# atomicarchitects/equiformer

Hardware: NVIDIA H100
Metric: edges/sec fwd+bwd, QM9 Lmax=2 batch (higher is better)
Workload: dtype f32

## Files before the change

equiformer_b200/csrc/eqf_fused.cu:

```cuda
#include <cuda.h>
#include <cuda_runtime.h>

#include <cstdint>
#include <mutex>
#include <string>
#include <vector>

#include "eqf_common.cuh"
#include "eqf_tc.cuh"

namespace eqf {
namespace fused {

using namespace tc;

constexpr int BM = 128;
constexpr int BKT = kKTile;
constexpr int kRowBytes = BKT * 4;
constexpr int kProducerWarp = 4;
constexpr int kHelperWarp0 = 6, kHelperWarps = 2, kHelperThreads = kHelperWarps * 32;
constexpr int kConsumerWarps = 8;
constexpr int kDtpWarp0 = 12, kDtpWarps = 16, kDtpSets = 2, kDtpSetWarps = kDtpWarps / kDtpSets;
constexpr int kDtpSetThreads = kDtpSetWarps * 32;
constexpr int kThreads = (kDtpWarp0 + kDtpWarps) * 32;
constexpr int kMaxBN = 64;
constexpr int kMaxPaths = 16;
constexpr int kMaxTileEdges = 136;
constexpr int kMetaInts = 2 * kMaxTileEdges;
constexpr int kMaxStages = 8;
constexpr int kMaxKTiles = 32;

struct FPath {
  int d1, d2;
  int xb, mul;
  int y_off, w_off;
  int cg_off;
  int koff;
  int m_off;
  unsigned long long nz;
};

struct FArgs {
  const float* x[EQF_MAX_BLOCKS];
  const float* x2[EQF_MAX_BLOCKS];
  const long long* src;
  const long long* dst;
  const float* y;
  const float* w;
  const float* w_offset;
  const float* cg;
  float* C;
  long long ldc;
  long long E, M;
  int d_y, W, w_shared, d3, n_paths, m_row, K, N;
  int n_tile, n_blocks;
  long long m_blocks;
  long long* dbg;
  int n_op, n_raw, op_bytes, w_tile_off, w_box_rows, tab_bytes, m_buf_floats, y_buf_floats, cg_floats;
  unsigned char kt_path[kMaxKTiles];
  FPath paths[kMaxPaths];
};

__device__ __forceinline__ void stamp(const FArgs& a, int role, int& n) {
  if (a.dbg != nullptr && blockIdx.x == 0 && n < 2048) a.dbg[role * 2048 + n] = clock64();
  ++n;
}


template <int BN>
struct FSmem {
  static constexpr int kABytes = BM * kRowBytes;
  static constexpr int kBBytes = BN * kRowBytes;
  static constexpr int kBarBytes = 1024;
  static constexpr int kBudget = 227 * 1024 - 1024;
};

__device__ __forceinline__ float4 ld4(const float* p) { return __ldg(reinterpret_cast<const float4*>(p)); }
__device__ __forceinline__ void addv(float4& a, const float4& b) { a.x += b.x; a.y += b.y; a.z += b.z; a.w += b.w; }
__device__ __forceinline__ void mulv(float4& a, const float4& b) { a.x *= b.x; a.y *= b.y; a.z *= b.z; a.w *= b.w; }
__device__ __forceinline__ void fs(float4& a, const float4& x, float m) {
  a.x = fmaf(x.x, m, a.x); a.y = fmaf(x.y, m, a.y); a.z = fmaf(x.z, m, a.z); a.w = fmaf(x.w, m, a.w);
}

struct Ring {
  int n, idx;
  uint32_t ph;
  __device__ __forceinline__ Ring(int n_) : n(n_), idx(0), ph(0) {}
  __device__ __forceinline__ void next() { if (++idx == n) { idx = 0; ph ^= 1u; } }
};

struct KtWaits { uint64_t* raw_free; uint32_t raw_ph; uint64_t* op_full; uint32_t op_ph; };

template <int D1, int D3, bool DIAG>
__device__ __forceinline__ void dtp_ktile(const FArgs& a, const FPath& p, int ch0, int t, long long e0, int n_e, long long row0,
                                          const int* __restrict__ src_s, const int* __restrict__ dst_s, uint32_t m_addr,
                                          uint32_t raw_addr, uint32_t w_tile, const KtWaits& wt) {
  constexpr int NM = (D1 * D3 + 3) / 4;
  const int c8 = t & 7;
  const int ch = ch0 + c8 * 4;
  const bool gather = a.src != nullptr;
  const float* xa = a.x[p.xb];
  const float* xb = a.x2[p.xb];
  const long long row_floats = (long long)D1 * p.mul;
  float4 woff = make_float4(0.f, 0.f, 0.f, 0.f);
  if (a.w_offset != nullptr) woff = ld4(a.w_offset + p.w_off + ch);
  bool waited = false;
  int el = t >> 3;
#pragma unroll 1
  do {
    const bool active = el < n_e;
    const int els = active ? el : 0;
    const long long e = e0 + els;
    const long long rs = gather ? (long long)src_s[els] : e;
    const float* xp = xa + rs * row_floats + ch;
    float4 x[D1];
#pragma unroll
    for (int i = 0; i < D1; ++i) x[i] = ld4(xp + i * p.mul);
    if (xb != nullptr) {
      const float* xq = xb + (long long)dst_s[els] * row_floats + ch;
      float4 x2[D1];
#pragma unroll
      for (int i = 0; i < D1; ++i) x2[i] = ld4(xq + i * p.mul);
#pragma unroll
      for (int i = 0; i < D1; ++i) addv(x[i], x2[i]);
    }
    if (!waited) {
      waited = true;
      mbar_wait_hint(wt.raw_free, wt.raw_ph);
      if (wt.op_full) mbar_wait_hint(wt.op_full, wt.op_ph);
    }
    if (!active) break;
    float4 wv = w_tile != 0 ? lds128(w_tile + (uint32_t)el * 128u + (uint32_t)c8 * 16u) : ld4(a.w + p.w_off + ch);
    addv(wv, woff);
    float m[NM * 4];
    const uint32_t ma = m_addr + (uint32_t)(el * a.m_row + p.m_off) * 4u;
#pragma unroll
    for (int q = 0; q < NM; ++q) {
      const float4 v = lds128(ma + (uint32_t)q * 16u);
      m[4 * q] = v.x; m[4 * q + 1] = v.y; m[4 * q + 2] = v.z; m[4 * q + 3] = v.w;
    }
    float4 f[D3];
    if constexpr (DIAG) {
#pragma unroll
      for (int k = 0; k < D3; ++k) {
        f[k] = x[k];
        mulv(f[k], wv);
        f[k].x *= m[k * D3 + k]; f[k].y *= m[k * D3 + k]; f[k].z *= m[k * D3 + k]; f[k].w *= m[k * D3 + k];
      }
    } else {
#pragma unroll
      for (int k = 0; k < D3; ++k) f[k] = make_float4(0.f, 0.f, 0.f, 0.f);
#pragma unroll
      for (int i = 0; i < D1; ++i) {
#pragma unroll
        for (int k = 0; k < D3; ++k) fs(f[k], x[i], m[i * D3 + k]);
      }
#pragma unroll
      for (int k = 0; k < D3; ++k) mulv(f[k], wv);
    }
    const int rbase = (int)(e * D3 - row0);
#pragma unroll
    for (int k = 0; k < D3; ++k) {
      const int row = rbase + k;
      if ((unsigned)row < (unsigned)BM) sts128(raw_addr + (uint32_t)row * 128u + (uint32_t)((c8 ^ (row & 7)) << 4), f[k]);
    }
    el += kDtpSetThreads / 8;
  } while (el < n_e);
}

template <int D3>
__device__ __forceinline__ void dtp_ktile_d1(const FArgs& a, const FPath& p, int ch0, int t, long long e0, int n_e, long long row0,
                                             const int* src_s, const int* dst_s, uint32_t m_addr, uint32_t raw_addr,
                                             uint32_t w_tile, const KtWaits& wt) {
  if (p.d2 == 1 && p.d1 == D3) {
    dtp_ktile<D3, D3, true>(a, p, ch0, t, e0, n_e, row0, src_s, dst_s, m_addr, raw_addr, w_tile, wt);
    return;
  }
  switch (p.d1) {
    case 1: dtp_ktile<1, D3, false>(a, p, ch0, t, e0, n_e, row0, src_s, dst_s, m_addr, raw_addr, w_tile, wt); break;
    case 3: dtp_ktile<3, D3, false>(a, p, ch0, t, e0, n_e, row0, src_s, dst_s, m_addr, raw_addr, w_tile, wt); break;
    case 5: dtp_ktile<5, D3, false>(a, p, ch0, t, e0, n_e, row0, src_s, dst_s, m_addr, raw_addr, w_tile, wt); break;
    default: dtp_ktile<7, D3, false>(a, p, ch0, t, e0, n_e, row0, src_s, dst_s, m_addr, raw_addr, w_tile, wt); break;
  }
}


template <int BN, int D3>
__global__ void __launch_bounds__(kThreads, 1)
dtp_gemm_fwd_kernel(const __grid_constant__ CUtensorMap map_bhi, const __grid_constant__ CUtensorMap map_blo,
                    const __grid_constant__ CUtensorMap map_w, const __grid_constant__ FArgs a) {
  using S = FSmem<BN>;
  const int n_op = a.n_op, n_raw = a.n_raw;
  extern __shared__ uint8_t smem_raw[];
  uint8_t* smem = reinterpret_cast<uint8_t*>((reinterpret_cast<uintptr_t>(smem_raw) + 1023) & ~uintptr_t(1023));
  uint8_t* op_base = smem;
  uint8_t* raw_base = smem + (size_t)n_op * a.op_bytes;
  uint8_t* tab_base = raw_base + (size_t)n_raw * S::kABytes;
  int4* mdesc = reinterpret_cast<int4*>(tab_base + 2 * a.tab_bytes);
  float* cg_s = reinterpret_cast<float*>(reinterpret_cast<uint8_t*>(mdesc) + ((a.m_row * 16 + 127) & ~127));
  uint64_t* bars = reinterpret_cast<uint64_t*>(reinterpret_cast<uint8_t*>(cg_s) + ((a.cg_floats * 4 + 127) & ~127));
  uint64_t* op_full = bars;
  uint64_t* op_empty = bars + kMaxStages;
  uint64_t* raw_ready = bars + 2 * kMaxStages;
  uint64_t* raw_free = bars + 3 * kMaxStages;
  uint64_t* tab_ready = bars + 4 * kMaxStages;
  uint64_t* tab_free = tab_ready + 2;

  const int warp = threadIdx.x >> 5, lane = threadIdx.x & 31;
  const int k_tiles = a.K / BKT;
  constexpr int d3 = D3;
  const long long n_tiles_total = a.m_blocks * a.n_blocks;
  const bool w_tma = !a.w_shared;

  if (threadIdx.x == kProducerWarp * 32) {
    prefetch_map(&map_bhi); prefetch_map(&map_blo);
    if (w_tma) prefetch_map(&map_w);
    for (int s = 0; s < kMaxStages; ++s) {
      mbar_init(&op_full[s], 1);
      mbar_init(&op_empty[s], kConsumerWarps);
      mbar_init(&raw_ready[s], kDtpSetWarps);
      mbar_init(&raw_free[s], kConsumerWarps);
    }
    for (int b = 0; b < 2; ++b) {
      mbar_init(&tab_ready[b], kHelperWarps);
      mbar_init(&tab_free[b], kDtpWarps);
    }
    asm volatile("fence.mbarrier_init.release.cluster;" ::: "memory");
  }
  __syncthreads();

  if (warp < 4 || (warp >= 8 && warp < kDtpWarp0)) {
    reg_alloc<80>();
    const int row_wg = (warp < 4 ? 0 : 64) + (warp & 3) * 16;
    const bool stamper = threadIdx.x == 0;
    Ring op(n_op), raw(n_raw);
    int n_stamp = 0;
    for (long long tile = blockIdx.x; tile < n_tiles_total; tile += gridDim.x) {
      const long long mb = tile / a.n_blocks;
      const int nb = (int)(tile % a.n_blocks);
      float acc[BN / 2];
#pragma unroll
      for (int i = 0; i < BN / 2; ++i) acc[i] = 0.f;
      for (int kt = 0; kt < k_tiles; ++kt, op.next(), raw.next()) {
        mbar_wait_hint(&op_full[op.idx], op.ph);
        mbar_wait_hint(&raw_ready[raw.idx], raw.ph);
        if (stamper) stamp(a, 1, n_stamp);
        const uint32_t raw_tile = smem_u32(raw_base + (size_t)raw.idx * S::kABytes);
        const uint32_t st = smem_u32(op_base + (size_t)op.idx * a.op_bytes);
#pragma unroll
        for (int half = 0; half < 2; ++half) {
          uint32_t hi[8], lo[8];
          load_a_split(raw_tile, row_wg, lane, hi, lo, 2 * half);
          if (half == 1) {
            __syncwarp();
            if (lane == 0) mbar_arrive(&raw_free[raw.idx]);
          }
          mma_ktile_3xtf32<BN>(acc, hi, lo, st, st + S::kBBytes, 2 * half);
          wgmma_wait<0>();
        }
        __syncwarp();
        if (lane == 0) mbar_arrive(&op_empty[op.idx]);
        if (stamper) stamp(a, 1, n_stamp);
      }
      store_acc<BN>(acc, a.C, a.ldc, mb * BM + row_wg, a.M, nb * BN, a.N, lane, false);
      if (stamper) stamp(a, 3, n_stamp);
    }
  } else if (warp < 8) {
    reg_dealloc<56>();
    if (warp == kProducerWarp) {
      if (lane == 0) {
        Ring op(n_op);
        int n_stamp = 0;
        const uint32_t tx = (uint32_t)(2 * S::kBBytes) + (w_tma ? (uint32_t)(a.w_box_rows * kRowBytes) : 0u);
        for (long long tile = blockIdx.x; tile < n_tiles_total; tile += gridDim.x) {
          const long long mb = tile / a.n_blocks;
          const int nb = (int)(tile % a.n_blocks);
          const int e0 = (int)((mb * BM) / d3);
          for (int kt = 0; kt < k_tiles; ++kt, op.next()) {
            mbar_wait_hint(&op_empty[op.idx], op.ph ^ 1);
            stamp(a, 0, n_stamp);
            uint8_t* st = op_base + (size_t)op.idx * a.op_bytes;
            mbar_expect_tx(&op_full[op.idx], tx);
            tma_load_2d(st, &map_bhi, kt * BKT, nb * BN, &op_full[op.idx]);
            tma_load_2d(st + S::kBBytes, &map_blo, kt * BKT, nb * BN, &op_full[op.idx]);
            if (w_tma) {
              const FPath& p = a.paths[a.kt_path[kt]];
              tma_load_2d(st + a.w_tile_off, &map_w, p.w_off + (kt * BKT - p.koff), e0, &op_full[op.idx]);
            }
          }
        }
      }
    } else if (warp >= kHelperWarp0) {
      const int ht = threadIdx.x - kHelperWarp0 * 32;
      const int m_row = a.m_row, d_y = a.d_y;
      {
        int off = 0;
        for (int pi = 0; pi < a.n_paths; ++pi) {
          const FPath& p = a.paths[pi];
          const int n = p.d1 * p.d2 * d3;
          for (int i = ht; i < n; i += kHelperThreads) cg_s[off + i] = __ldg(a.cg + p.cg_off + i);
          off += n;
        }
        for (int q = ht; q < m_row; q += kHelperThreads) {
          int pi = 0, cg0 = 0;
          for (int j = 1; j < a.n_paths; ++j) if (q >= a.paths[j].m_off) pi = j;
          for (int j = 0; j < pi; ++j) cg0 += a.paths[j].d1 * a.paths[j].d2 * d3;
          const FPath& p = a.paths[pi];
          const int r = q - p.m_off;
          const int i = r / d3, k = r - i * d3;
          if (i < p.d1) mdesc[q] = make_int4(cg0 + i * p.d2 * d3 + k, p.y_off, p.d2, 0);
          else mdesc[q] = make_int4(0, 0, 0, 0);
        }
        named_barrier(2, kHelperThreads);
      }
      const uint32_t cg_addr = smem_u32(cg_s);
      uint32_t tile_it = 0;
      int n_stamp = 0;
      for (long long tile = blockIdx.x; tile < n_tiles_total; tile += gridDim.x, ++tile_it) {
        const long long mb = tile / a.n_blocks;
        const long long row0 = mb * BM;
        const long long e0 = row0 / d3;
        long long e1 = (row0 + BM - 1) / d3 + 1;
        if (e1 > a.E) e1 = a.E;
        const int n_e = (int)(e1 - e0);
        const int b = tile_it & 1;
        mbar_wait_hint(&tab_free[b], ((tile_it >> 1) & 1) ^ 1);
        if (ht == 0) stamp(a, 5, n_stamp);
        float* mw = reinterpret_cast<float*>(tab_base + b * a.tab_bytes);
        float* ybuf = mw + a.m_buf_floats;
        int* ss = reinterpret_cast<int*>(ybuf + a.y_buf_floats);
        int* ds = ss + kMaxTileEdges;
        if (a.src != nullptr) {
          for (int i = ht; i < n_e; i += kHelperThreads) {
            ss[i] = (int)a.src[e0 + i];
            ds[i] = a.dst != nullptr ? (int)a.dst[e0 + i] : 0;
          }
        }
        for (int i = ht; i < n_e * d_y; i += kHelperThreads) ybuf[i] = __ldg(a.y + e0 * d_y + i);
        named_barrier(2, kHelperThreads);
        const uint32_t y_addr = smem_u32(ybuf);
        for (int q = ht; q < m_row; q += kHelperThreads) {
          const int4 dsc = mdesc[q];
          float cgr[kMaxD];
#pragma unroll
          for (int j = 0; j < kMaxD; ++j) cgr[j] = j < dsc.z ? lds32(cg_addr + (uint32_t)(dsc.x + j * d3) * 4u) : 0.f;
#pragma unroll 4
          for (int el = 0; el < n_e; ++el) {
            const uint32_t ya = y_addr + (uint32_t)(el * d_y + dsc.y) * 4u;
            float m = 0.f;
#pragma unroll
            for (int j = 0; j < kMaxD; ++j)
              if (j < dsc.z) m = fmaf(cgr[j], lds32(ya + (uint32_t)j * 4u), m);
            mw[el * m_row + q] = m;
          }
        }
        __syncwarp();
        if (lane == 0) mbar_arrive(&tab_ready[b]);
        if (ht == 0) stamp(a, 5, n_stamp);
      }
    }
  } else {
    const int dt = threadIdx.x - kDtpWarp0 * 32;
    const int set = (warp - kDtpWarp0) / kDtpSetWarps;
    const int t = dt - set * kDtpSetThreads;
    Ring op(n_op), raw(n_raw);
    uint32_t it = 0, tile_it = 0;
    int n_stamp = 0;
    const bool stamper = (t == 0 && set == 0);
    for (long long tile = blockIdx.x; tile < n_tiles_total; tile += gridDim.x, ++tile_it) {
      const long long mb = tile / a.n_blocks;
      const long long row0 = mb * BM;
      const long long e0 = row0 / d3;
      long long e1 = (row0 + BM - 1) / d3 + 1;
      if (e1 > a.E) e1 = a.E;
      const int n_e = (int)(e1 - e0);
      const int b = tile_it & 1;
      mbar_wait_hint(&tab_ready[b], (tile_it >> 1) & 1);
      if (stamper) stamp(a, 4, n_stamp);
      const float* mw = reinterpret_cast<const float*>(tab_base + b * a.tab_bytes);
      const float* ybuf = mw + a.m_buf_floats;
      const int* src_s = reinterpret_cast<const int*>(ybuf + a.y_buf_floats);
      const int* dst_s = src_s + kMaxTileEdges;
      const uint32_t m_addr = smem_u32(mw);
      for (int kt = 0; kt < k_tiles; ++kt, ++it, op.next(), raw.next()) {
        if ((int)(it & 1) != set) continue;
        const FPath& p = a.paths[a.kt_path[kt]];
        const int ch0 = kt * BKT - p.koff;
        const uint32_t raw_addr = smem_u32(raw_base + (size_t)raw.idx * S::kABytes);
        const uint32_t w_tile = w_tma ? smem_u32(op_base + (size_t)op.idx * a.op_bytes) + (uint32_t)a.w_tile_off : 0u;
        KtWaits wt;
        wt.raw_free = &raw_free[raw.idx]; wt.raw_ph = raw.ph ^ 1;
        wt.op_full = w_tma ? &op_full[op.idx] : nullptr; wt.op_ph = op.ph;
        if (stamper) stamp(a, 4, n_stamp);
        dtp_ktile_d1<D3>(a, p, ch0, t, e0, n_e, row0, src_s, dst_s, m_addr, raw_addr, w_tile, wt);
        __syncwarp();
        if (lane == 0) mbar_arrive(&raw_ready[raw.idx]);
        if (stamper) stamp(a, 4, n_stamp);
      }
      __syncwarp();
      if (lane == 0) mbar_arrive(&tab_free[b]);
    }
  }
}

template <int D1, int D3>
__device__ __forceinline__ void group_ktile(const FArgs& a, const FPath& p, int ch0, int el, int c8, long long e,
                                            const float* __restrict__ me, float* __restrict__ out) {
  const int ch = ch0 + c8 * 4;
  float4 wv = ld4(a.w + (a.w_shared ? 0 : e * a.W) + p.w_off + ch);
  if (a.w_offset != nullptr) addv(wv, ld4(a.w_offset + p.w_off + ch));
  const long long row_floats = (long long)D1 * p.mul;
  const long long rs = a.src != nullptr ? a.src[e] : e;
  const float* xp = a.x[p.xb] + rs * row_floats + ch;
  float4 x[D1];
#pragma unroll
  for (int i = 0; i < D1; ++i) x[i] = ld4(xp + i * p.mul);
  if (a.x2[p.xb] != nullptr) {
    const float* xq = a.x2[p.xb] + a.dst[e] * row_floats + ch;
#pragma unroll
    for (int i = 0; i < D1; ++i) addv(x[i], ld4(xq + i * p.mul));
  }
#pragma unroll
  for (int i = 0; i < D1; ++i) mulv(x[i], wv);
#pragma unroll
  for (int k = 0; k < D3; ++k) {
    float4 f = make_float4(0.f, 0.f, 0.f, 0.f);
#pragma unroll
    for (int i = 0; i < D1; ++i)
      if ((p.nz >> (i * D3 + k)) & 1ull) fs(f, x[i], me[i * D3 + k]);
    *reinterpret_cast<float4*>(out + (e * D3 + k) * a.K + p.koff + ch) = f;
  }
}

template <int D3>
__global__ void __launch_bounds__(256) dtp_group_forward_kernel(const __grid_constant__ FArgs a, float* __restrict__ out) {
  extern __shared__ float msm[];
  const int t = threadIdx.x, el = t >> 3, c8 = t & 7;
  const int m_row = a.m_row;
  for (long long eb = (long long)blockIdx.x * 32; eb < a.E; eb += (long long)gridDim.x * 32) {
    const int n_e = (int)((a.E - eb) < 32 ? (a.E - eb) : 32);
    __syncthreads();
    for (int idx = t; idx < n_e * m_row; idx += 256) {
      const int ee = idx / m_row, q = idx - ee * m_row;
      int pi = 0;
      for (int j = 1; j < a.n_paths; ++j) if (q >= a.paths[j].m_off) pi = j;
      const FPath& p = a.paths[pi];
      const int r = q - p.m_off;
      const int i = r / D3, k = r - i * D3;
      const float* cg = a.cg + p.cg_off + i * p.d2 * D3 + k;
      const float* yv = a.y + (eb + ee) * a.d_y + p.y_off;
      float m = 0.f;
      for (int j = 0; j < (i < p.d1 ? p.d2 : 0); ++j) m = fmaf(__ldg(cg + j * D3), __ldg(yv + j), m);
      msm[idx] = m;
    }
    __syncthreads();
    if (el < n_e) {
      const long long e = eb + el;
      for (int pi = 0; pi < a.n_paths; ++pi) {
        const FPath& p = a.paths[pi];
        const float* me = msm + el * m_row + p.m_off;
        for (int ch0 = 0; ch0 < p.mul; ch0 += BKT) {
          switch (p.d1) {
            case 1: group_ktile<1, D3>(a, p, ch0, el, c8, e, me, out); break;
            case 3: group_ktile<3, D3>(a, p, ch0, el, c8, e, me, out); break;
            case 5: group_ktile<5, D3>(a, p, ch0, el, c8, e, me, out); break;
            default: group_ktile<7, D3>(a, p, ch0, el, c8, e, me, out); break;
          }
        }
      }
    }
  }
}

__global__ void split_transpose_kernel(const float* __restrict__ w, long long ldw, float* __restrict__ hi,
                                       float* __restrict__ lo, long long N, long long K) {
  const long long n_el = N * K;
  for (long long i = (long long)blockIdx.x * blockDim.x + threadIdx.x; i < n_el; i += (long long)gridDim.x * blockDim.x) {
    const long long n = i / K, k = i - n * K;
    const float v = w[k * ldw + n];
    const float h = tf32_rn(v);
    hi[i] = h;
    lo[i] = tf32_rn(v - h);
  }
}

template <int BN, int D3>
static int launch_fwd_d3(const CUtensorMap& mh, const CUtensorMap& ml, const CUtensorMap& mw, FArgs& a, cudaStream_t s) {
  using S = FSmem<BN>;
  const int n_e_max = BM / a.d3 + 2;
  a.w_box_rows = a.w_shared ? 0 : n_e_max;
  a.w_tile_off = 2 * S::kBBytes;
  a.op_bytes = (a.w_tile_off + a.w_box_rows * kRowBytes + 1023) & ~1023;
  a.m_buf_floats = (n_e_max * a.m_row + 31) & ~31;
  a.y_buf_floats = (n_e_max * a.d_y + 31) & ~31;
  a.cg_floats = 0;
  for (int i = 0; i < a.n_paths; ++i) a.cg_floats += a.paths[i].d1 * a.paths[i].d2 * a.d3;
  a.tab_bytes = ((a.m_buf_floats + a.y_buf_floats) * 4 + kMetaInts * 4 + 127) & ~127;
  const int fixed = 2 * a.tab_bytes + ((a.m_row * 16 + 127) & ~127) + ((a.cg_floats * 4 + 127) & ~127) + S::kBarBytes;
  int n_raw = 0, n_op = 0;
  for (int r = 4; r >= 2 && n_raw == 0; --r) {
    const int o = (S::kBudget - fixed - r * S::kABytes) / a.op_bytes;
    if (o >= r || (r == 2 && o >= 2)) { n_raw = r; n_op = o; }
  }
  if (n_raw == 0) { set_error("fused DTP: the tile does not fit shared memory"); return EQF_ERR_UNSUPPORTED; }
  if (n_op > kMaxStages) n_op = kMaxStages;
  a.n_raw = n_raw; a.n_op = n_op;
  const int total = n_op * a.op_bytes + n_raw * S::kABytes + fixed + 1024;
  static std::mutex mtx;
  static int attr_bytes = 0;
  {
    std::lock_guard<std::mutex> lock(mtx);
    if (total > attr_bytes) {
      cudaError_t e = cudaFuncSetAttribute(dtp_gemm_fwd_kernel<BN, D3>, cudaFuncAttributeMaxDynamicSharedMemorySize, total);
      if (e != cudaSuccess) return check_cuda(e, "dtp_gemm_fwd smem attribute");
      attr_bytes = total;
    }
  }
  const int sms = device_sms();
  const long long tiles = a.m_blocks * a.n_blocks;
  const int grid = (int)(tiles < sms ? tiles : sms);
  dtp_gemm_fwd_kernel<BN, D3><<<grid, kThreads, total, s>>>(mh, ml, mw, a);
  return check_cuda(cudaGetLastError(), "dtp_gemm_fwd_kernel launch");
}

template <int BN>
static int launch_fwd(const CUtensorMap& mh, const CUtensorMap& ml, const CUtensorMap& mw, FArgs& a, cudaStream_t s) {
  switch (a.d3) {
    case 1: return launch_fwd_d3<BN, 1>(mh, ml, mw, a, s);
    case 3: return launch_fwd_d3<BN, 3>(mh, ml, mw, a, s);
    case 5: return launch_fwd_d3<BN, 5>(mh, ml, mw, a, s);
    default: return launch_fwd_d3<BN, 7>(mh, ml, mw, a, s);
  }
}

static int collect_paths(const EqfPlan* plan, int group, FArgs& a) {
  const PlanHdr& h = plan->hdr;
  if (group < 0 || group >= h.n_out) { set_error("fused DTP: output group out of range"); return EQF_ERR_INVALID; }
  const PathDev* pd = reinterpret_cast<const PathDev*>(plan->blob.data() + h.off_paths);
  std::vector<const PathDev*> ps;
  for (int p = 0; p < h.n_paths; ++p) if (pd[p].og == group) ps.push_back(&pd[p]);
  for (size_t i = 0; i < ps.size(); ++i)
    for (size_t j = i; j > 0 && ps[j]->koff < ps[j - 1]->koff; --j) std::swap(ps[j], ps[j - 1]);
  if (ps.empty() || (int)ps.size() > kMaxPaths) { set_error("fused DTP: unsupported number of paths in the group"); return EQF_ERR_UNSUPPORTED; }
  int koff = 0, m_off = 0;
  for (size_t i = 0; i < ps.size(); ++i) {
    const PathDev& s = *ps[i];
    if (s.d1 > kMaxD || s.d2 > kMaxD || s.d3 > kMaxD) {
      set_error("fused DTP: degree-4 paths are not supported (2l+1 <= 7)");
      return EQF_ERR_UNSUPPORTED;
    }
    if (s.koff != koff || s.mul % BKT != 0) {
      set_error("fused DTP: group channels must be covered by paths of multiplicity % 32 == 0");
      return EQF_ERR_UNSUPPORTED;
    }
    FPath& f = a.paths[i];
    f.d1 = s.d1; f.d2 = s.d2; f.xb = s.xb; f.mul = s.mul; f.y_off = s.y_off; f.w_off = s.w_off; f.cg_off = s.cg_off;
    f.koff = s.koff; f.m_off = m_off;
    f.nz = 0;
    const float* cgp = reinterpret_cast<const float*>(plan->blob.data() + h.off_cg) + s.cg_off;
    for (int ii = 0; ii < s.d1; ++ii)
      for (int kk = 0; kk < s.d3; ++kk) {
        bool any = false;
        for (int jj = 0; jj < s.d2; ++jj) any = any || cgp[(ii * s.d2 + jj) * s.d3 + kk] != 0.0f;
        if (any) f.nz |= 1ull << (ii * s.d3 + kk);
      }
    for (int c = 0; c < s.mul / BKT; ++c) {
      if (koff / BKT + c >= kMaxKTiles) { set_error("fused DTP: output group wider than 1024 channels"); return EQF_ERR_UNSUPPORTED; }
      a.kt_path[koff / BKT + c] = (unsigned char)i;
    }
    koff += s.mul;
    m_off += (s.d1 * s.d3 + 3) & ~3;
  }
  a.n_paths = (int)ps.size();
  a.d3 = h.out_d[group];
  a.K = koff;
  a.m_row = m_off;
  if (koff != h.out_mul[group]) { set_error("fused DTP: paths do not cover the output group"); return EQF_ERR_INVALID; }
  if ((BM / a.d3 + 2) * a.m_row * 4 > 40 * 1024) { set_error("fused DTP: coupling blocks of a tile exceed shared memory"); return EQF_ERR_UNSUPPORTED; }
  return a.n_paths;
}

}
}

using namespace eqf;

extern "C" int eqf_dtp_linear_supported(const EqfPlan* plan, int32_t group) {
  if (plan == nullptr) return 0;
  fused::FArgs a;
  const PlanHdr& h = plan->hdr;
  for (int b = 0; b < h.n_in1; ++b) if (h.in1_mul[b] % 4 != 0) return 0;
  if (h.w_numel % 4 != 0) return 0;
  return fused::collect_paths(plan, group, a) > 0 ? 1 : 0;
}

static long long* g_fused_dbg = nullptr;
extern "C" void eqf_fused_set_timeline(long long* device_buffer) { g_fused_dbg = device_buffer; }

static int fill_fargs(const EqfPlan* plan, const EqfEdgeOperands* op, int64_t n_edges, int32_t group, eqf::fused::FArgs& a,
                      const char* who) {
  using namespace eqf::fused;
  if (plan == nullptr || op == nullptr) { set_error(std::string(who) + ": null plan / operands"); return EQF_ERR_INVALID; }
  if (!op->y || !op->w) { set_error(std::string(who) + ": null pointer"); return EQF_ERR_INVALID; }
  int rc = ensure_device(plan);
  if (rc != EQF_OK) return rc;
  const PlanHdr& h = plan->hdr;
  rc = collect_paths(plan, group, a);
  if (rc < 0) return rc;
  if ((((uintptr_t)op->w | (uintptr_t)op->w_offset) & 15) || (h.w_numel & 3)) {
    set_error(std::string(who) + ": weights must be 16-byte aligned, weight_numel % 4 == 0");
    return EQF_ERR_INVALID;
  }
  for (int b = 0; b < EQF_MAX_BLOCKS; ++b) { a.x[b] = nullptr; a.x2[b] = nullptr; }
  for (int b = 0; b < h.n_in1; ++b) {
    if (op->x[b] == nullptr || ((uintptr_t)op->x[b] & 15) || ((uintptr_t)op->x2[b] & 15) || (h.in1_mul[b] & 3)) {
      set_error(std::string(who) + ": in1 blocks must be present, 16-byte aligned, multiplicities % 4 == 0");
      return EQF_ERR_INVALID;
    }
    a.x[b] = op->x[b];
    a.x2[b] = op->x2[b];
  }
  a.src = reinterpret_cast<const long long*>(op->src);
  a.dst = reinterpret_cast<const long long*>(op->dst);
  if (a.x2[0] != nullptr && (a.src == nullptr || a.dst == nullptr)) { set_error(std::string(who) + ": x2 needs src and dst"); return EQF_ERR_INVALID; }
  a.y = op->y; a.w = op->w; a.w_offset = op->w_offset; a.w_shared = op->w_shared;
  if (a.w_shared && a.w_offset != nullptr) { set_error(std::string(who) + ": w_offset needs per-edge weights"); return EQF_ERR_INVALID; }
  a.cg = reinterpret_cast<const float*>(plan->d_blob + h.off_cg);
  a.C = nullptr; a.ldc = 0;
  a.E = n_edges; a.M = n_edges * a.d3; a.d_y = h.d_y; a.W = h.w_numel; a.N = 0;
  if (a.M > 0x7fffffffLL) { set_error(std::string(who) + ": too many rows"); return EQF_ERR_UNSUPPORTED; }
  a.n_tile = a.n_blocks = 0; a.m_blocks = 0;
  a.n_op = a.n_raw = a.op_bytes = a.w_tile_off = a.w_box_rows = a.tab_bytes = a.m_buf_floats = a.y_buf_floats = a.cg_floats = 0;
  a.dbg = g_fused_dbg;
  return EQF_OK;
}

extern "C" int eqf_dtp_group_forward(const EqfPlan* plan, const EqfEdgeOperands* op, int64_t n_edges, int32_t group,
                                     float* out, void* stream) {
  using namespace eqf::fused;
  if (n_edges <= 0) return EQF_OK;
  if (out == nullptr || ((uintptr_t)out & 15)) { set_error("eqf_dtp_group_forward: bad output pointer"); return EQF_ERR_INVALID; }
  FArgs a;
  int rc = fill_fargs(plan, op, n_edges, group, a, "eqf_dtp_group_forward");
  if (rc != EQF_OK) return rc;
  const size_t smem = (size_t)32 * a.m_row * sizeof(float);
  const long long blocks = (n_edges + 31) / 32;
  const int cap = device_sms() * 8;
  const int grid = (int)(blocks < cap ? blocks : cap);
  cudaStream_t s = (cudaStream_t)stream;
  switch (a.d3) {
    case 1: dtp_group_forward_kernel<1><<<grid, 256, smem, s>>>(a, out); break;
    case 3: dtp_group_forward_kernel<3><<<grid, 256, smem, s>>>(a, out); break;
    case 5: dtp_group_forward_kernel<5><<<grid, 256, smem, s>>>(a, out); break;
    default: dtp_group_forward_kernel<7><<<grid, 256, smem, s>>>(a, out); break;
  }
  return check_cuda(cudaGetLastError(), "dtp_group_forward_kernel launch");
}

extern "C" int eqf_dtp_linear_fwd(const EqfPlan* plan, const EqfEdgeOperands* op, int64_t n_edges, int32_t group,
                                  const float* Wt, int64_t N, int64_t ldw, float* C, int64_t ldc, float* split,
                                  void* stream) {
  using namespace eqf::fused;
  if (n_edges <= 0 || N <= 0) return EQF_OK;
  if (!Wt || !C || !split) { set_error("eqf_dtp_linear_fwd: null pointer"); return EQF_ERR_INVALID; }
  FArgs a;
  int rc = fill_fargs(plan, op, n_edges, group, a, "eqf_dtp_linear_fwd");
  if (rc != EQF_OK) return rc;
  const PlanHdr& h = plan->hdr;
  if ((((uintptr_t)C | (uintptr_t)split) & 15) || ((N | ldc) & 3) || ldc < N || ldw < N) {
    set_error("eqf_dtp_linear_fwd: operands must be 16-byte aligned, N and ldc multiples of 4");
    return EQF_ERR_INVALID;
  }
  a.N = (int)N;
  cudaStream_t s = (cudaStream_t)stream;
  const long long K = a.K;
  float* hi = split;
  float* lo = split + N * K;
  {
    const long long n = N * K;
    const unsigned blocks = (unsigned)((n + 255) / 256 < 1056 ? (n + 255) / 256 : 1056);
    split_transpose_kernel<<<blocks, 256, 0, s>>>(Wt, ldw, hi, lo, N, K);
  }
  if ((rc = check_cuda(cudaGetLastError(), "split_transpose_kernel launch")) != EQF_OK) return rc;
  const int n_blocks = (int)((N + kMaxBN - 1) / kMaxBN);
  const int n_tile = (n_blocks == 1 && N <= 32) ? 32 : kMaxBN;
  a.n_tile = n_tile; a.n_blocks = n_blocks; a.m_blocks = (a.M + BM - 1) / BM;
  a.C = C; a.ldc = ldc;
  CUtensorMap mh, ml, mw;
  if ((rc = make_map_2d(&mh, hi, N, K, K, n_tile, BKT)) != EQF_OK) return rc;
  if ((rc = make_map_2d(&ml, lo, N, K, K, n_tile, BKT)) != EQF_OK) return rc;
  mw = mh;
  if (!a.w_shared && (rc = make_map_2d(&mw, a.w, n_edges, h.w_numel, h.w_numel, BM / a.d3 + 2, BKT, MapKind::kLinear)) != EQF_OK)
    return rc;
  if (n_tile == 32) return launch_fwd<32>(mh, ml, mw, a, s);
  return launch_fwd<64>(mh, ml, mw, a, s);
}
```

Before: 1.450 million.

## Reorder fused DTP-linear to GEMM on per-channel products then apply CG per edge

The kernel used to build per-row DTP products (x times CG-contracted y, D3 rows per edge) in shared memory before the tensor-core GEMM. It now runs the GEMM on per-edge x·w tiles (one row per edge, one k-tile per input component i1) and applies the CG/y contraction afterwards in registers of the consumer warps, accumulating D3 outputs per edge. This cuts the GEMM's M dimension by D3 and shrinks the DTP producer to 4 warps, but it repeats the GEMM per i1 component and may split columns into several passes. It also raises consumer register pressure (out[D3][CW/2]) and adds CG FMAs to the consumer warps.

```diff
diff --git a/equiformer_b200/csrc/eqf_fused.cu b/equiformer_b200/csrc/eqf_fused.cu
--- a/equiformer_b200/csrc/eqf_fused.cu
+++ b/equiformer_b200/csrc/eqf_fused.cu
@@ -20,21 +20,21 @@
 constexpr int kProducerWarp = 4;
 constexpr int kHelperWarp0 = 6, kHelperWarps = 2, kHelperThreads = kHelperWarps * 32;
 constexpr int kConsumerWarps = 8;
-constexpr int kDtpWarp0 = 12, kDtpWarps = 16, kDtpSets = 2, kDtpSetWarps = kDtpWarps / kDtpSets;
-constexpr int kDtpSetThreads = kDtpSetWarps * 32;
+constexpr int kDtpWarp0 = 12, kDtpWarps = 4, kDtpThreads = kDtpWarps * 32;
 constexpr int kThreads = (kDtpWarp0 + kDtpWarps) * 32;
+constexpr int kEdgesPerThread = BM / (kDtpThreads / 8);
 constexpr int kMaxBN = 64;
 constexpr int kMaxPaths = 16;
-constexpr int kMaxTileEdges = 136;
-constexpr int kMetaInts = 2 * kMaxTileEdges;
 constexpr int kMaxStages = 8;
-constexpr int kMaxKTiles = 32;
+
+__host__ __device__ constexpr int col_pass(int bn, int d3) { return d3 * bn <= 192 ? bn : 32; }
 
 struct FPath {
   int d1, d2;
   int xb, mul;
   int y_off, w_off;
   int cg_off;
+  int cs_off;
   int koff;
   int m_off;
   unsigned long long nz;
@@ -56,8 +56,7 @@
   int n_tile, n_blocks;
   long long m_blocks;
   long long* dbg;
-  int n_op, n_raw, op_bytes, w_tile_off, w_box_rows, tab_bytes, m_buf_floats, y_buf_floats, cg_floats;
-  unsigned char kt_path[kMaxKTiles];
+  int n_op, n_raw, op_bytes, w_tile_off, w_box_rows, tab_bytes, y_buf_floats, cg_floats;
   FPath paths[kMaxPaths];
 };
 
@@ -67,10 +66,10 @@
 }
 
 
-template <int BN>
+template <int CW>
 struct FSmem {
   static constexpr int kABytes = BM * kRowBytes;
-  static constexpr int kBBytes = BN * kRowBytes;
+  static constexpr int kBBytes = CW * kRowBytes;
   static constexpr int kBarBytes = 1024;
   static constexpr int kBudget = 227 * 1024 - 1024;
 };
@@ -89,115 +88,24 @@
   __device__ __forceinline__ void next() { if (++idx == n) { idx = 0; ph ^= 1u; } }
 };
 
-struct KtWaits { uint64_t* raw_free; uint32_t raw_ph; uint64_t* op_full; uint32_t op_ph; };
-
-template <int D1, int D3, bool DIAG>
-__device__ __forceinline__ void dtp_ktile(const FArgs& a, const FPath& p, int ch0, int t, long long e0, int n_e, long long row0,
-                                          const int* __restrict__ src_s, const int* __restrict__ dst_s, uint32_t m_addr,
-                                          uint32_t raw_addr, uint32_t w_tile, const KtWaits& wt) {
-  constexpr int NM = (D1 * D3 + 3) / 4;
-  const int c8 = t & 7;
-  const int ch = ch0 + c8 * 4;
-  const bool gather = a.src != nullptr;
-  const float* xa = a.x[p.xb];
-  const float* xb = a.x2[p.xb];
-  const long long row_floats = (long long)D1 * p.mul;
-  float4 woff = make_float4(0.f, 0.f, 0.f, 0.f);
-  if (a.w_offset != nullptr) woff = ld4(a.w_offset + p.w_off + ch);
-  bool waited = false;
-  int el = t >> 3;
-#pragma unroll 1
-  do {
-    const bool active = el < n_e;
-    const int els = active ? el : 0;
-    const long long e = e0 + els;
-    const long long rs = gather ? (long long)src_s[els] : e;
-    const float* xp = xa + rs * row_floats + ch;
-    float4 x[D1];
-#pragma unroll
-    for (int i = 0; i < D1; ++i) x[i] = ld4(xp + i * p.mul);
-    if (xb != nullptr) {
-      const float* xq = xb + (long long)dst_s[els] * row_floats + ch;
-      float4 x2[D1];
-#pragma unroll
-      for (int i = 0; i < D1; ++i) x2[i] = ld4(xq + i * p.mul);
-#pragma unroll
-      for (int i = 0; i < D1; ++i) addv(x[i], x2[i]);
-    }
-    if (!waited) {
-      waited = true;
-      mbar_wait_hint(wt.raw_free, wt.raw_ph);
-      if (wt.op_full) mbar_wait_hint(wt.op_full, wt.op_ph);
-    }
-    if (!active) break;
-    float4 wv = w_tile != 0 ? lds128(w_tile + (uint32_t)el * 128u + (uint32_t)c8 * 16u) : ld4(a.w + p.w_off + ch);
-    addv(wv, woff);
-    float m[NM * 4];
-    const uint32_t ma = m_addr + (uint32_t)(el * a.m_row + p.m_off) * 4u;
-#pragma unroll
-    for (int q = 0; q < NM; ++q) {
-      const float4 v = lds128(ma + (uint32_t)q * 16u);
-      m[4 * q] = v.x; m[4 * q + 1] = v.y; m[4 * q + 2] = v.z; m[4 * q + 3] = v.w;
-    }
-    float4 f[D3];
-    if constexpr (DIAG) {
-#pragma unroll
-      for (int k = 0; k < D3; ++k) {
-        f[k] = x[k];
-        mulv(f[k], wv);
-        f[k].x *= m[k * D3 + k]; f[k].y *= m[k * D3 + k]; f[k].z *= m[k * D3 + k]; f[k].w *= m[k * D3 + k];
-      }
-    } else {
-#pragma unroll
-      for (int k = 0; k < D3; ++k) f[k] = make_float4(0.f, 0.f, 0.f, 0.f);
-#pragma unroll
-      for (int i = 0; i < D1; ++i) {
-#pragma unroll
-        for (int k = 0; k < D3; ++k) fs(f[k], x[i], m[i * D3 + k]);
-      }
-#pragma unroll
-      for (int k = 0; k < D3; ++k) mulv(f[k], wv);
-    }
-    const int rbase = (int)(e * D3 - row0);
-#pragma unroll
-    for (int k = 0; k < D3; ++k) {
-      const int row = rbase + k;
-      if ((unsigned)row < (unsigned)BM) sts128(raw_addr + (uint32_t)row * 128u + (uint32_t)((c8 ^ (row & 7)) << 4), f[k]);
-    }
-    el += kDtpSetThreads / 8;
-  } while (el < n_e);
-}
-
-template <int D3>
-__device__ __forceinline__ void dtp_ktile_d1(const FArgs& a, const FPath& p, int ch0, int t, long long e0, int n_e, long long row0,
-                                             const int* src_s, const int* dst_s, uint32_t m_addr, uint32_t raw_addr,
-                                             uint32_t w_tile, const KtWaits& wt) {
-  if (p.d2 == 1 && p.d1 == D3) {
-    dtp_ktile<D3, D3, true>(a, p, ch0, t, e0, n_e, row0, src_s, dst_s, m_addr, raw_addr, w_tile, wt);
-    return;
-  }
-  switch (p.d1) {
-    case 1: dtp_ktile<1, D3, false>(a, p, ch0, t, e0, n_e, row0, src_s, dst_s, m_addr, raw_addr, w_tile, wt); break;
-    case 3: dtp_ktile<3, D3, false>(a, p, ch0, t, e0, n_e, row0, src_s, dst_s, m_addr, raw_addr, w_tile, wt); break;
-    case 5: dtp_ktile<5, D3, false>(a, p, ch0, t, e0, n_e, row0, src_s, dst_s, m_addr, raw_addr, w_tile, wt); break;
-    default: dtp_ktile<7, D3, false>(a, p, ch0, t, e0, n_e, row0, src_s, dst_s, m_addr, raw_addr, w_tile, wt); break;
-  }
-}
-
+__device__ __forceinline__ int n_passes(const FArgs& a, int nb, int bn, int cw) {
+  const int left = (a.N - nb * bn + cw - 1) / cw;
+  return left < bn / cw ? left : bn / cw;
+}
 
 template <int BN, int D3>
 __global__ void __launch_bounds__(kThreads, 1)
 dtp_gemm_fwd_kernel(const __grid_constant__ CUtensorMap map_bhi, const __grid_constant__ CUtensorMap map_blo,
                     const __grid_constant__ CUtensorMap map_w, const __grid_constant__ FArgs a) {
-  using S = FSmem<BN>;
+  constexpr int CW = col_pass(BN, D3);
+  using S = FSmem<CW>;
   const int n_op = a.n_op, n_raw = a.n_raw;
   extern __shared__ uint8_t smem_raw[];
   uint8_t* smem = reinterpret_cast<uint8_t*>((reinterpret_cast<uintptr_t>(smem_raw) + 1023) & ~uintptr_t(1023));
   uint8_t* op_base = smem;
   uint8_t* raw_base = smem + (size_t)n_op * a.op_bytes;
   uint8_t* tab_base = raw_base + (size_t)n_raw * S::kABytes;
-  int4* mdesc = reinterpret_cast<int4*>(tab_base + 2 * a.tab_bytes);
-  float* cg_s = reinterpret_cast<float*>(reinterpret_cast<uint8_t*>(mdesc) + ((a.m_row * 16 + 127) & ~127));
+  float* cg_s = reinterpret_cast<float*>(tab_base + 2 * a.tab_bytes);
   uint64_t* bars = reinterpret_cast<uint64_t*>(reinterpret_cast<uint8_t*>(cg_s) + ((a.cg_floats * 4 + 127) & ~127));
   uint64_t* op_full = bars;
   uint64_t* op_empty = bars + kMaxStages;
@@ -207,8 +115,6 @@
   uint64_t* tab_free = tab_ready + 2;
 
   const int warp = threadIdx.x >> 5, lane = threadIdx.x & 31;
-  const int k_tiles = a.K / BKT;
-  constexpr int d3 = D3;
   const long long n_tiles_total = a.m_blocks * a.n_blocks;
   const bool w_tma = !a.w_shared;
 
@@ -218,55 +124,105 @@
     for (int s = 0; s < kMaxStages; ++s) {
       mbar_init(&op_full[s], 1);
       mbar_init(&op_empty[s], kConsumerWarps);
-      mbar_init(&raw_ready[s], kDtpSetWarps);
+      mbar_init(&raw_ready[s], kDtpWarps);
       mbar_init(&raw_free[s], kConsumerWarps);
     }
     for (int b = 0; b < 2; ++b) {
       mbar_init(&tab_ready[b], kHelperWarps);
-      mbar_init(&tab_free[b], kDtpWarps);
+      mbar_init(&tab_free[b], kDtpWarps + kConsumerWarps);
     }
     asm volatile("fence.mbarrier_init.release.cluster;" ::: "memory");
   }
   __syncthreads();
 
   if (warp < 4 || (warp >= 8 && warp < kDtpWarp0)) {
-    reg_alloc<80>();
+    reg_alloc<160>();
     const int row_wg = (warp < 4 ? 0 : 64) + (warp & 3) * 16;
+    const int r0 = row_wg + (lane >> 2);
     const bool stamper = threadIdx.x == 0;
+    const uint32_t cg_addr = smem_u32(cg_s);
     Ring op(n_op), raw(n_raw);
     int n_stamp = 0;
-    for (long long tile = blockIdx.x; tile < n_tiles_total; tile += gridDim.x) {
+    uint32_t tile_it = 0;
+    float z[CW / 2];
+#pragma unroll
+    for (int i = 0; i < CW / 2; ++i) z[i] = 0.f;
+    for (long long tile = blockIdx.x; tile < n_tiles_total; tile += gridDim.x, ++tile_it) {
       const long long mb = tile / a.n_blocks;
       const int nb = (int)(tile % a.n_blocks);
-      float acc[BN / 2];
-#pragma unroll
-      for (int i = 0; i < BN / 2; ++i) acc[i] = 0.f;
-      for (int kt = 0; kt < k_tiles; ++kt, op.next(), raw.next()) {
-        mbar_wait_hint(&op_full[op.idx], op.ph);
-        mbar_wait_hint(&raw_ready[raw.idx], raw.ph);
-        if (stamper) stamp(a, 1, n_stamp);
-        const uint32_t raw_tile = smem_u32(raw_base + (size_t)raw.idx * S::kABytes);
-        const uint32_t st = smem_u32(op_base + (size_t)op.idx * a.op_bytes);
-#pragma unroll
-        for (int half = 0; half < 2; ++half) {
-          uint32_t hi[8], lo[8];
-          load_a_split(raw_tile, row_wg, lane, hi, lo, 2 * half);
-          if (half == 1) {
-            __syncwarp();
-            if (lane == 0) mbar_arrive(&raw_free[raw.idx]);
+      const int b = tile_it & 1;
+      mbar_wait_hint(&tab_ready[b], (tile_it >> 1) & 1);
+      const uint32_t y_addr = smem_u32(tab_base + b * a.tab_bytes);
+      const int n_pass = n_passes(a, nb, BN, CW);
+      for (int pass = 0; pass < n_pass; ++pass) {
+        float out[D3][CW / 2];
+#pragma unroll
+        for (int k = 0; k < D3; ++k)
+#pragma unroll
+          for (int i = 0; i < CW / 2; ++i) out[k][i] = 0.f;
+        for (int pi = 0; pi < a.n_paths; ++pi) {
+          const FPath& p = a.paths[pi];
+          const int n_c = p.mul / BKT;
+          for (int i1 = 0; i1 < p.d1; ++i1) {
+            for (int c = 0; c < n_c; ++c, op.next(), raw.next()) {
+              mbar_wait_hint(&op_full[op.idx], op.ph);
+              mbar_wait_hint(&raw_ready[raw.idx], raw.ph);
+              if (stamper) stamp(a, 1, n_stamp);
+              const uint32_t raw_tile = smem_u32(raw_base + (size_t)raw.idx * S::kABytes);
+              const uint32_t st = smem_u32(op_base + (size_t)op.idx * a.op_bytes);
+#pragma unroll
+              for (int half = 0; half < 2; ++half) {
+                uint32_t hi[8], lo[8];
+                load_a_split(raw_tile, row_wg, lane, hi, lo, 2 * half);
+                if (half == 1) {
+                  __syncwarp();
+                  if (lane == 0) mbar_arrive(&raw_free[raw.idx]);
+                }
+                if (half == 0 && c == 0) mma_ktile_3xtf32<CW, true>(z, hi, lo, st, st + S::kBBytes, 0);
+                else mma_ktile_3xtf32<CW, false>(z, hi, lo, st, st + S::kBBytes, 2 * half);
+                wgmma_wait<0>();
+              }
+              __syncwarp();
+              if (lane == 0) mbar_arrive(&op_empty[op.idx]);
+              if (stamper) stamp(a, 1, n_stamp);
+            }
+            float m[2][D3];
+#pragma unroll
+            for (int h = 0; h < 2; ++h)
+#pragma unroll
+              for (int k = 0; k < D3; ++k) m[h][k] = 0.f;
+            const uint32_t cg_row = cg_addr + (uint32_t)(p.cs_off + i1 * p.d2 * D3) * 4u;
+            const uint32_t ya0 = y_addr + (uint32_t)(r0 * a.d_y + p.y_off) * 4u;
+            const uint32_t ya1 = ya0 + (uint32_t)(8 * a.d_y) * 4u;
+#pragma unroll
+            for (int j = 0; j < kMaxD; ++j) {
+              if (j < p.d2) {
+                const float y0 = lds32(ya0 + (uint32_t)j * 4u), y1 = lds32(ya1 + (uint32_t)j * 4u);
+#pragma unroll
+                for (int k = 0; k < D3; ++k) {
+                  const float cgv = lds32(cg_row + (uint32_t)(j * D3 + k) * 4u);
+                  m[0][k] = fmaf(cgv, y0, m[0][k]);
+                  m[1][k] = fmaf(cgv, y1, m[1][k]);
+                }
+              }
+            }
+#pragma unroll
+            for (int k = 0; k < D3; ++k)
+#pragma unroll
+              for (int i = 0; i < CW / 2; ++i) out[k][i] = fmaf(m[(i >> 1) & 1][k], z[i], out[k][i]);
           }
-          mma_ktile_3xtf32<BN>(acc, hi, lo, st, st + S::kBBytes, 2 * half);
-          wgmma_wait<0>();
         }
-        __syncwarp();
-        if (lane == 0) mbar_arrive(&op_empty[op.idx]);
-        if (stamper) stamp(a, 1, n_stamp);
-      }
-      store_acc<BN>(acc, a.C, a.ldc, mb * BM + row_wg, a.M, nb * BN, a.N, lane, false);
-      if (stamper) stamp(a, 3, n_stamp);
+        const int col0 = nb * BN + pass * CW;
+#pragma unroll
+        for (int k = 0; k < D3; ++k)
+          store_acc<CW>(out[k], a.C + k * a.ldc, a.ldc * D3, mb * BM + row_wg, a.E, col0, a.N, lane, false);
+        if (stamper) stamp(a, 3, n_stamp);
+      }
+      __syncwarp();
+      if (lane == 0) mbar_arrive(&tab_free[b]);
     }
   } else if (warp < 8) {
-    reg_dealloc<56>();
+    reg_dealloc<40>();
     if (warp == kProducerWarp) {
       if (lane == 0) {
         Ring op(n_op);
@@ -275,61 +231,46 @@
         for (long long tile = blockIdx.x; tile < n_tiles_total; tile += gridDim.x) {
           const long long mb = tile / a.n_blocks;
           const int nb = (int)(tile % a.n_blocks);
-          const int e0 = (int)((mb * BM) / d3);
-          for (int kt = 0; kt < k_tiles; ++kt, op.next()) {
-            mbar_wait_hint(&op_empty[op.idx], op.ph ^ 1);
-            stamp(a, 0, n_stamp);
-            uint8_t* st = op_base + (size_t)op.idx * a.op_bytes;
-            mbar_expect_tx(&op_full[op.idx], tx);
-            tma_load_2d(st, &map_bhi, kt * BKT, nb * BN, &op_full[op.idx]);
-            tma_load_2d(st + S::kBBytes, &map_blo, kt * BKT, nb * BN, &op_full[op.idx]);
-            if (w_tma) {
-              const FPath& p = a.paths[a.kt_path[kt]];
-              tma_load_2d(st + a.w_tile_off, &map_w, p.w_off + (kt * BKT - p.koff), e0, &op_full[op.idx]);
+          const int e0 = (int)(mb * BM);
+          const int n_pass = n_passes(a, nb, BN, CW);
+          for (int pass = 0; pass < n_pass; ++pass) {
+            const int col0 = nb * BN + pass * CW;
+            for (int pi = 0; pi < a.n_paths; ++pi) {
+              const FPath& p = a.paths[pi];
+              for (int i1 = 0; i1 < p.d1; ++i1) {
+                for (int ch0 = 0; ch0 < p.mul; ch0 += BKT, op.next()) {
+                  mbar_wait_hint(&op_empty[op.idx], op.ph ^ 1);
+                  stamp(a, 0, n_stamp);
+                  uint8_t* st = op_base + (size_t)op.idx * a.op_bytes;
+                  mbar_expect_tx(&op_full[op.idx], tx);
+                  tma_load_2d(st, &map_bhi, p.koff + ch0, col0, &op_full[op.idx]);
+                  tma_load_2d(st + S::kBBytes, &map_blo, p.koff + ch0, col0, &op_full[op.idx]);
+                  if (w_tma) tma_load_2d(st + a.w_tile_off, &map_w, p.w_off + ch0, e0, &op_full[op.idx]);
+                }
+              }
             }
           }
         }
       }
     } else if (warp >= kHelperWarp0) {
       const int ht = threadIdx.x - kHelperWarp0 * 32;
-      const int m_row = a.m_row, d_y = a.d_y;
-      {
-        int off = 0;
-        for (int pi = 0; pi < a.n_paths; ++pi) {
-          const FPath& p = a.paths[pi];
-          const int n = p.d1 * p.d2 * d3;
-          for (int i = ht; i < n; i += kHelperThreads) cg_s[off + i] = __ldg(a.cg + p.cg_off + i);
-          off += n;
-        }
-        for (int q = ht; q < m_row; q += kHelperThreads) {
-          int pi = 0, cg0 = 0;
-          for (int j = 1; j < a.n_paths; ++j) if (q >= a.paths[j].m_off) pi = j;
-          for (int j = 0; j < pi; ++j) cg0 += a.paths[j].d1 * a.paths[j].d2 * d3;
-          const FPath& p = a.paths[pi];
-          const int r = q - p.m_off;
-          const int i = r / d3, k = r - i * d3;
-          if (i < p.d1) mdesc[q] = make_int4(cg0 + i * p.d2 * d3 + k, p.y_off, p.d2, 0);
-          else mdesc[q] = make_int4(0, 0, 0, 0);
-        }
-        named_barrier(2, kHelperThreads);
-      }
-      const uint32_t cg_addr = smem_u32(cg_s);
+      const int d_y = a.d_y;
+      for (int pi = 0; pi < a.n_paths; ++pi) {
+        const FPath& p = a.paths[pi];
+        const int n = p.d1 * p.d2 * D3;
+        for (int i = ht; i < n; i += kHelperThreads) cg_s[p.cs_off + i] = __ldg(a.cg + p.cg_off + i);
+      }
       uint32_t tile_it = 0;
       int n_stamp = 0;
       for (long long tile = blockIdx.x; tile < n_tiles_total; tile += gridDim.x, ++tile_it) {
-        const long long mb = tile / a.n_blocks;
-        const long long row0 = mb * BM;
-        const long long e0 = row0 / d3;
-        long long e1 = (row0 + BM - 1) / d3 + 1;
-        if (e1 > a.E) e1 = a.E;
-        const int n_e = (int)(e1 - e0);
+        const long long e0 = (tile / a.n_blocks) * BM;
+        const int n_e = (int)(a.E - e0 < BM ? a.E - e0 : BM);
         const int b = tile_it & 1;
         mbar_wait_hint(&tab_free[b], ((tile_it >> 1) & 1) ^ 1);
         if (ht == 0) stamp(a, 5, n_stamp);
-        float* mw = reinterpret_cast<float*>(tab_base + b * a.tab_bytes);
-        float* ybuf = mw + a.m_buf_floats;
+        float* ybuf = reinterpret_cast<float*>(tab_base + b * a.tab_bytes);
         int* ss = reinterpret_cast<int*>(ybuf + a.y_buf_floats);
-        int* ds = ss + kMaxTileEdges;
+        int* ds = ss + BM;
         if (a.src != nullptr) {
           for (int i = ht; i < n_e; i += kHelperThreads) {
             ss[i] = (int)a.src[e0 + i];
@@ -337,65 +278,77 @@
           }
         }
         for (int i = ht; i < n_e * d_y; i += kHelperThreads) ybuf[i] = __ldg(a.y + e0 * d_y + i);
-        named_barrier(2, kHelperThreads);
-        const uint32_t y_addr = smem_u32(ybuf);
-        for (int q = ht; q < m_row; q += kHelperThreads) {
-          const int4 dsc = mdesc[q];
-          float cgr[kMaxD];
-#pragma unroll
-          for (int j = 0; j < kMaxD; ++j) cgr[j] = j < dsc.z ? lds32(cg_addr + (uint32_t)(dsc.x + j * d3) * 4u) : 0.f;
-#pragma unroll 4
-          for (int el = 0; el < n_e; ++el) {
-            const uint32_t ya = y_addr + (uint32_t)(el * d_y + dsc.y) * 4u;
-            float m = 0.f;
-#pragma unroll
-            for (int j = 0; j < kMaxD; ++j)
-              if (j < dsc.z) m = fmaf(cgr[j], lds32(ya + (uint32_t)j * 4u), m);
-            mw[el * m_row + q] = m;
-          }
-        }
         __syncwarp();
         if (lane == 0) mbar_arrive(&tab_ready[b]);
         if (ht == 0) stamp(a, 5, n_stamp);
       }
     }
   } else {
-    const int dt = threadIdx.x - kDtpWarp0 * 32;
-    const int set = (warp - kDtpWarp0) / kDtpSetWarps;
-    const int t = dt - set * kDtpSetThreads;
+    reg_alloc<152>();
+    const int t = threadIdx.x - kDtpWarp0 * 32;
+    const int c8 = t & 7, el0 = t >> 3;
+    const bool gather = a.src != nullptr;
+    const bool stamper = t == 0;
     Ring op(n_op), raw(n_raw);
-    uint32_t it = 0, tile_it = 0;
+    uint32_t tile_it = 0;
     int n_stamp = 0;
-    const bool stamper = (t == 0 && set == 0);
     for (long long tile = blockIdx.x; tile < n_tiles_total; tile += gridDim.x, ++tile_it) {
-      const long long mb = tile / a.n_blocks;
-      const long long row0 = mb * BM;
-      const long long e0 = row0 / d3;
-      long long e1 = (row0 + BM - 1) / d3 + 1;
-      if (e1 > a.E) e1 = a.E;
-      const int n_e = (int)(e1 - e0);
+      const long long e0 = (tile / a.n_blocks) * BM;
+      const int nb = (int)(tile % a.n_blocks);
+      const int n_e = (int)(a.E - e0 < BM ? a.E - e0 : BM);
       const int b = tile_it & 1;
       mbar_wait_hint(&tab_ready[b], (tile_it >> 1) & 1);
-      if (stamper) stamp(a, 4, n_stamp);
-      const float* mw = reinterpret_cast<const float*>(tab_base + b * a.tab_bytes);
-      const float* ybuf = mw + a.m_buf_floats;
-      const int* src_s = reinterpret_cast<const int*>(ybuf + a.y_buf_floats);
-      const int* dst_s = src_s + kMaxTileEdges;
-      const uint32_t m_addr = smem_u32(mw);
-      for (int kt = 0; kt < k_tiles; ++kt, ++it, op.next(), raw.next()) {
-        if ((int)(it & 1) != set) continue;
-        const FPath& p = a.paths[a.kt_path[kt]];
-        const int ch0 = kt * BKT - p.koff;
-        const uint32_t raw_addr = smem_u32(raw_base + (size_t)raw.idx * S::kABytes);
-        const uint32_t w_tile = w_tma ? smem_u32(op_base + (size_t)op.idx * a.op_bytes) + (uint32_t)a.w_tile_off : 0u;
-        KtWaits wt;
-        wt.raw_free = &raw_free[raw.idx]; wt.raw_ph = raw.ph ^ 1;
-        wt.op_full = w_tma ? &op_full[op.idx] : nullptr; wt.op_ph = op.ph;
-        if (stamper) stamp(a, 4, n_stamp);
-        dtp_ktile_d1<D3>(a, p, ch0, t, e0, n_e, row0, src_s, dst_s, m_addr, raw_addr, w_tile, wt);
-        __syncwarp();
-        if (lane == 0) mbar_arrive(&raw_ready[raw.idx]);
-        if (stamper) stamp(a, 4, n_stamp);
+      const int* src_s = reinterpret_cast<const int*>(tab_base + b * a.tab_bytes + a.y_buf_floats * 4);
+      const int* dst_s = src_s + BM;
+      int rs[kEdgesPerThread], rd[kEdgesPerThread];
+#pragma unroll
+      for (int j = 0; j < kEdgesPerThread; ++j) {
+        const int el = el0 + j * (kDtpThreads / 8);
+        const int els = el < n_e ? el : 0;
+        rs[j] = gather ? src_s[els] : (int)(e0 + els);
+        rd[j] = gather && a.dst != nullptr ? dst_s[els] : 0;
+      }
+      const int n_pass = n_passes(a, nb, BN, CW);
+      for (int pass = 0; pass < n_pass; ++pass) {
+        for (int pi = 0; pi < a.n_paths; ++pi) {
+          const FPath& p = a.paths[pi];
+          const long long row_floats = (long long)p.d1 * p.mul;
+          const float* xa = a.x[p.xb];
+          const float* xb = a.x2[p.xb];
+          for (int i1 = 0; i1 < p.d1; ++i1) {
+            for (int ch0 = 0; ch0 < p.mul; ch0 += BKT, op.next(), raw.next()) {
+              if (stamper) stamp(a, 4, n_stamp);
+              const int col = i1 * p.mul + ch0 + c8 * 4;
+              float4 x[kEdgesPerThread];
+#pragma unroll
+              for (int j = 0; j < kEdgesPerThread; ++j) x[j] = ld4(xa + (long long)rs[j] * row_floats + col);
+              if (xb != nullptr) {
+#pragma unroll
+                for (int j = 0; j < kEdgesPerThread; ++j) addv(x[j], ld4(xb + (long long)rd[j] * row_floats + col));
+              }
+              float4 woff = make_float4(0.f, 0.f, 0.f, 0.f);
+              if (a.w_offset != nullptr) woff = ld4(a.w_offset + p.w_off + ch0 + c8 * 4);
+              if (!w_tma) addv(woff, ld4(a.w + p.w_off + ch0 + c8 * 4));
+              mbar_wait_hint(&raw_free[raw.idx], raw.ph ^ 1);
+              if (w_tma) mbar_wait_hint(&op_full[op.idx], op.ph);
+              const uint32_t raw_addr = smem_u32(raw_base + (size_t)raw.idx * S::kABytes);
+              const uint32_t w_tile = smem_u32(op_base + (size_t)op.idx * a.op_bytes) + (uint32_t)a.w_tile_off;
+#pragma unroll
+              for (int j = 0; j < kEdgesPerThread; ++j) {
+                const int el = el0 + j * (kDtpThreads / 8);
+                float4 wv = woff;
+                if (w_tma) addv(wv, lds128(w_tile + (uint32_t)el * 128u + (uint32_t)c8 * 16u));
+                float4 f = x[j];
+                mulv(f, wv);
+                if (el >= n_e) f = make_float4(0.f, 0.f, 0.f, 0.f);
+                sts128(raw_addr + (uint32_t)el * 128u + (uint32_t)((c8 ^ (el & 7)) << 4), f);
+              }
+              __syncwarp();
+              if (lane == 0) mbar_arrive(&raw_ready[raw.idx]);
+              if (stamper) stamp(a, 4, n_stamp);
+            }
+          }
+        }
       }
       __syncwarp();
       if (lane == 0) mbar_arrive(&tab_free[b]);
@@ -486,17 +439,16 @@
 
 template <int BN, int D3>
 static int launch_fwd_d3(const CUtensorMap& mh, const CUtensorMap& ml, const CUtensorMap& mw, FArgs& a, cudaStream_t s) {
-  using S = FSmem<BN>;
-  const int n_e_max = BM / a.d3 + 2;
-  a.w_box_rows = a.w_shared ? 0 : n_e_max;
+  constexpr int CW = col_pass(BN, D3);
+  using S = FSmem<CW>;
+  a.w_box_rows = a.w_shared ? 0 : BM;
   a.w_tile_off = 2 * S::kBBytes;
   a.op_bytes = (a.w_tile_off + a.w_box_rows * kRowBytes + 1023) & ~1023;
-  a.m_buf_floats = (n_e_max * a.m_row + 31) & ~31;
-  a.y_buf_floats = (n_e_max * a.d_y + 31) & ~31;
+  a.y_buf_floats = (BM * a.d_y + 31) & ~31;
   a.cg_floats = 0;
   for (int i = 0; i < a.n_paths; ++i) a.cg_floats += a.paths[i].d1 * a.paths[i].d2 * a.d3;
-  a.tab_bytes = ((a.m_buf_floats + a.y_buf_floats) * 4 + kMetaInts * 4 + 127) & ~127;
-  const int fixed = 2 * a.tab_bytes + ((a.m_row * 16 + 127) & ~127) + ((a.cg_floats * 4 + 127) & ~127) + S::kBarBytes;
+  a.tab_bytes = (a.y_buf_floats * 4 + 2 * BM * 4 + 127) & ~127;
+  const int fixed = 2 * a.tab_bytes + ((a.cg_floats * 4 + 127) & ~127) + S::kBarBytes;
   int n_raw = 0, n_op = 0;
   for (int r = 4; r >= 2 && n_raw == 0; --r) {
     const int o = (S::kBudget - fixed - r * S::kABytes) / a.op_bytes;
@@ -542,7 +494,7 @@
   for (size_t i = 0; i < ps.size(); ++i)
     for (size_t j = i; j > 0 && ps[j]->koff < ps[j - 1]->koff; --j) std::swap(ps[j], ps[j - 1]);
   if (ps.empty() || (int)ps.size() > kMaxPaths) { set_error("fused DTP: unsupported number of paths in the group"); return EQF_ERR_UNSUPPORTED; }
-  int koff = 0, m_off = 0;
+  int koff = 0, m_off = 0, cs_off = 0;
   for (size_t i = 0; i < ps.size(); ++i) {
     const PathDev& s = *ps[i];
     if (s.d1 > kMaxD || s.d2 > kMaxD || s.d3 > kMaxD) {
@@ -564,12 +516,10 @@
         for (int jj = 0; jj < s.d2; ++jj) any = any || cgp[(ii * s.d2 + jj) * s.d3 + kk] != 0.0f;
         if (any) f.nz |= 1ull << (ii * s.d3 + kk);
       }
-    for (int c = 0; c < s.mul / BKT; ++c) {
-      if (koff / BKT + c >= kMaxKTiles) { set_error("fused DTP: output group wider than 1024 channels"); return EQF_ERR_UNSUPPORTED; }
-      a.kt_path[koff / BKT + c] = (unsigned char)i;
-    }
+    f.cs_off = cs_off;
     koff += s.mul;
     m_off += (s.d1 * s.d3 + 3) & ~3;
+    cs_off += s.d1 * s.d2 * s.d3;
   }
   a.n_paths = (int)ps.size();
   a.d3 = h.out_d[group];
@@ -630,7 +580,7 @@
   a.E = n_edges; a.M = n_edges * a.d3; a.d_y = h.d_y; a.W = h.w_numel; a.N = 0;
   if (a.M > 0x7fffffffLL) { set_error(std::string(who) + ": too many rows"); return EQF_ERR_UNSUPPORTED; }
   a.n_tile = a.n_blocks = 0; a.m_blocks = 0;
-  a.n_op = a.n_raw = a.op_bytes = a.w_tile_off = a.w_box_rows = a.tab_bytes = a.m_buf_floats = a.y_buf_floats = a.cg_floats = 0;
+  a.n_op = a.n_raw = a.op_bytes = a.w_tile_off = a.w_box_rows = a.tab_bytes = a.y_buf_floats = a.cg_floats = 0;
   a.dbg = g_fused_dbg;
   return EQF_OK;
 }
@@ -684,13 +634,14 @@
   if ((rc = check_cuda(cudaGetLastError(), "split_transpose_kernel launch")) != EQF_OK) return rc;
   const int n_blocks = (int)((N + kMaxBN - 1) / kMaxBN);
   const int n_tile = (n_blocks == 1 && N <= 32) ? 32 : kMaxBN;
-  a.n_tile = n_tile; a.n_blocks = n_blocks; a.m_blocks = (a.M + BM - 1) / BM;
+  a.n_tile = n_tile; a.n_blocks = n_blocks; a.m_blocks = (n_edges + BM - 1) / BM;
   a.C = C; a.ldc = ldc;
   CUtensorMap mh, ml, mw;
-  if ((rc = make_map_2d(&mh, hi, N, K, K, n_tile, BKT)) != EQF_OK) return rc;
-  if ((rc = make_map_2d(&ml, lo, N, K, K, n_tile, BKT)) != EQF_OK) return rc;
+  const int cw = col_pass(n_tile, a.d3);
+  if ((rc = make_map_2d(&mh, hi, N, K, K, cw, BKT)) != EQF_OK) return rc;
+  if ((rc = make_map_2d(&ml, lo, N, K, K, cw, BKT)) != EQF_OK) return rc;
   mw = mh;
-  if (!a.w_shared && (rc = make_map_2d(&mw, a.w, n_edges, h.w_numel, h.w_numel, BM / a.d3 + 2, BKT, MapKind::kLinear)) != EQF_OK)
+  if (!a.w_shared && (rc = make_map_2d(&mw, a.w, n_edges, h.w_numel, h.w_numel, BM, BKT, MapKind::kLinear)) != EQF_OK)
     return rc;
   if (n_tile == 32) return launch_fwd<32>(mh, ml, mw, a, s);
   return launch_fwd<64>(mh, ml, mw, a, s);
```

Result: no change. 1.449 million (median of 6 runs) (-0.1%).
